# microsoft/XPretrain

Hardware: AMD Instinct MI355X
Metric: video-text pairs/sec (higher is better)
Workload: dtype bf16; 1 GPU; CLIP-ViP ViT-B/16 video-text contrastive train step (fwd+loss+bwd+grad-sync+clip+AdamW), 12 frames 224^2, 32 text tokens, local batch 8, BASELINE configs[1]; global_batch=8, parallelism=dp1, gemm_cu_budget=256, grad_wire=fp32, forced_one_rank_collectives=False, video_forward_chains=2, optimizer_overlaps_next_forward_from_layer=3, launch=eager

## Files before the change

include/xpretrain_hip.h:

```cpp
#ifndef XPRETRAIN_HIP_H
#define XPRETRAIN_HIP_H

#include <stddef.h>
#include <stdint.h>

#ifdef __cplusplus
extern "C" {
#endif

#define XP_ABI_VERSION 1

enum { XP_BF16 = 0, XP_F32 = 1 };
enum { XP_OK = 0, XP_ERR_ARG = -1, XP_ERR_LAUNCH = -2, XP_ERR_UNSUPPORTED = -3 };

int xp_abi_version(void);
const char* xp_last_error(void);

enum {
  XP_EPI_NONE = 0,
  XP_EPI_BIAS = 1,
  XP_EPI_BIAS_QSCALE = 2,
  XP_EPI_BIAS_GELU = 3,
  XP_EPI_BIAS_RESID = 4,
  XP_EPI_GELU_BWD = 5,
// ... 321 lines not shown
  const float* ln1_w; const float* ln1_b; const float* bqkv; const float* bo;
  const float* ln2_w; const float* ln2_b; const float* b1; const float* b2;
  void* h1; void* kv; float* mean1; float* rstd1;
  void* h1p; void* q; void* attn_o; void* x2; void* h2; void* pre; void* act; void* x3;
  float* mean1p; float* rstd1p; float* mean2; float* rstd2; float* stats;
  void* workspace; size_t workspace_bytes;
  const float* side_in; float* side_out; float* side_x2;
} XpLayerPooledFwd;
size_t xp_encoder_layer_pooled_fwd_workspace_bytes(const XpLayerDims* dims);
int xp_encoder_layer_pooled_fwd(const XpLayerPooledFwd* args, void* stream);

typedef struct XpLayerPooledBwd {
  XpLayerDims dims;
  const void* x; const void* h1; const void* kv; const void* h1p; const void* q; const void* attn_o; const void* x2;
  const void* h2; const void* pre; const void* act; const void* Wqkv; const void* Wo; const void* W1; const void* W2;
  const float* ln1_w; const float* ln2_w; const float* mean1; const float* rstd1; const float* mean1p; const float* rstd1p;
  const float* mean2; const float* rstd2; const float* stats;
  const void* dx3;
  void* dx;
  float* dln1_w; float* dln1_b; float* dwqkv; float* dbqkv; float* dwo; float* dbo;
  float* dln2_w; float* dln2_b; float* dw1; float* db1; float* dw2; float* db2;
  void* workspace; size_t workspace_bytes;
  const float* side_in; const float* side_x2;
} XpLayerPooledBwd;
size_t xp_encoder_layer_pooled_bwd_workspace_bytes(const XpLayerDims* dims);
int xp_encoder_layer_pooled_bwd(const XpLayerPooledBwd* args, void* stream);
void* xp_side_stream(void);

int xp_debug_set_gemm_trace(void* device_buffer);
int xp_debug_gemm_timer_arm(int64_t M, int64_t N, int64_t K, int32_t epilogue, int32_t a_kstrided, int32_t b_kstrided, int32_t split_k,
                            int32_t max_launches);
int32_t xp_debug_gemm_timer_read(float* ms, int32_t cap);
int xp_debug_set_attn_trace(void* device_buffer);
int xp_debug_gemm_occupancy(int lds_bytes);
enum { XP_GEMM_FAMILY_256 = 0,
       XP_GEMM_FAMILY_DIRECT = 1,
       XP_GEMM_FAMILY_STAGED = 2,
       XP_GEMM_FAMILY_FRAMES = 3 };
enum { XP_GEMM_EPI_FAST = 0,
       XP_GEMM_EPI_ROW8 = 1,
       XP_GEMM_EPI_ROW4 = 2 };
typedef struct XpGemmPlanInfo {
  int32_t family, tile_rows;
  int32_t split, flat_split;
  int64_t k_per_split;
  int32_t tiles_m, tiles_n, group_n;
  int32_t epi_impl;
  int32_t grid[3];
  int32_t reserved;
  int64_t colsum_rows;
} XpGemmPlanInfo;
int xp_debug_gemm_plan(const XpGemmDesc* desc, XpGemmPlanInfo* out);
enum { XP_ATTN_KERNEL_FWD = 0,
       XP_ATTN_KERNEL_FWD3 = 1,
       XP_ATTN_KERNEL_FWD4 = 2,
       XP_ATTN_KERNEL_BWD_PAIR = 3,
       XP_ATTN_KERNEL_BWD5 = 4,
       XP_ATTN_KERNEL_F32 = 5 };
enum { XP_ATTN_OPTIN_BWD6 = 6 };
typedef struct XpAttnPlanInfo {
  int32_t kernel;
  int32_t grid, lds_bytes;
  int32_t reduce_grid;
  int32_t uses_counter;
  int32_t reserved;
  int64_t part[2], delta[2], dq[2], dkv[2], counter[2];
// ... 43 lines not shown
```

xpretrain_amd/csrc/attention.hip:

```cpp
#include "common.h"
#include <math.h>
#include <stdlib.h>
#include <string.h>
#include <type_traits>

namespace {

constexpr int DH = 64;
constexpr float F32_MIN = -3.4028234663852886e38f;

struct AP {
  const bf16_t* qkv; int64_t ldqkv;
  bf16_t* out; const bf16_t* dout; int64_t ldo;
  bf16_t* dqkv;
  float* stats;
  const int64_t* pad;
  int mode, B, H, S, M, N, L, R;
  int nq, nprob;
  float q_scale;
  float* ws0; float* ws1; float* ws2;
  unsigned long long* tr;
  float* cs; int cs_main;
};

// ... 395 lines not shown
  }
}

template <int NTL>
__device__ __forceinline__ void fwd3_walk(FwdState (&st)[F3T], const AP& p, int frame, const char* gK, const char* gV,
                                          const bf16x8 (&qf)[F3T][2], int ng, int kb0, bool corner, int lane) {
  int t0 = 0;
  for (; t0 + 4 <= ng && kb0 + (t0 + 4) * 16 <= p.R; t0 += 4) fwd3_step<4, NTL, false>(st, p, frame, gK, gV, qf, t0, corner, lane, kb0);
  if (t0 < ng) {
    if (ng - t0 == 1) {
      if (kb0 + ng * 16 > p.R) fwd3_step<1, NTL, true>(st, p, frame, gK, gV, qf, t0, corner, lane, kb0);
      else                     fwd3_step<1, NTL, false>(st, p, frame, gK, gV, qf, t0, corner, lane, kb0);
    } else {
      fwd3_step<4, NTL, true>(st, p, frame, gK, gV, qf, t0, corner, lane, kb0);
    }
  }
}
__device__ __forceinline__ void fwd3_finish(const FwdState (&st)[F3T], const AP& p, const Prob& pr, int prob, int tile0, int nt,
                                            int wave, int lane) {
#pragma unroll
  for (int i = 0; i < F3T; ++i)
    if (i < nt) fwd_finish_row(st[i], p, pr, prob, (tile0 + wave + F3W * i) * 16 + (lane & 15), lane >> 4);
}
template <int NTL>
__device__ __forceinline__ void fwd3_problem(const AP& p, const Prob& pr, int prob, const char* gK, const char* gV,
                                             const bf16x8 (&qf)[F3T][2], int nsub, int wave, int lane) {
  FwdState st[F3T];
#pragma unroll
  for (int i = 0; i < F3T; ++i) fwd_init(st[i], M_INIT);
  fwd3_walk<NTL>(st, p, pr.n, gK, gV, qf, nsub, 0, wave == 0, lane);
  fwd3_finish(st, p, pr, prob, 0, NTL, wave, lane);
}

__global__ __launch_bounds__(F3THR, 2) void attn_fwd3_kernel(AP p) {
  extern __shared__ __attribute__((aligned(16))) char smem[];
  const int tid = threadIdx.x, lane = tid & 63;
  const int wave = __builtin_amdgcn_readfirstlane(tid >> 6);
  const int nsub = (p.R + 15) / 16;
  const int nt = (nsub - wave + F3W - 1) / F3W;
  int prob = blockIdx.x;
  if (prob >= p.nprob) return;
  int cur = 0;
  bf16x8 qf[F3T][2], qn[F3T][2];
  {
    const Prob pr(p, prob);
    fwd3_stage_kv(smem, smem + FG * 128, p, pr, lane, wave, 0);
    fwd3_load_q(qf, p, pr, wave, lane, 0);
  }
  unsigned long long* tr = (p.tr && (int)blockIdx.x == (int)gridDim.x / 2 && (wave == 0 || wave == 7) && lane == 0)
                               ? p.tr + (wave ? 64 : 0) : nullptr;
  int it = 0;
  for (;;) {
    if (tr && it < 8) tr[it * 4 + 0] = __builtin_amdgcn_s_memtime();
    __syncthreads();
    if (tr && it < 8) tr[it * 4 + 1] = __builtin_amdgcn_s_memtime();
    const Prob pr(p, prob);
    const int next = prob + (int)gridDim.x;
    char* gK = smem + cur * F3_BUF;
    if (next < p.nprob) {
      const Prob pn(p, next);
      char* nK = smem + (cur ^ 1) * F3_BUF;
      fwd3_stage_kv(nK, nK + FG * 128, p, pn, lane, wave, 0);
      fwd3_load_q(qn, p, pn, wave, lane, 0);
    }
    if (tr && it < 8) tr[it * 4 + 2] = __builtin_amdgcn_s_memtime();
    if (nt == 2)      fwd3_problem<2>(p, pr, prob, gK, gK + FG * 128, qf, nsub, wave, lane);
    else if (nt == 1) fwd3_problem<1>(p, pr, prob, gK, gK + FG * 128, qf, nsub, wave, lane);
    if (tr && it < 8) tr[it * 4 + 3] = __builtin_amdgcn_s_memtime();
    ++it;
    if (next >= p.nprob) break;
#pragma unroll
    for (int i = 0; i < F3T; ++i)
#pragma unroll
      for (int kk = 0; kk < 2; ++kk) qf[i][kk] = qn[i][kk];
    prob = next; cur ^= 1;
  }
}

struct F4Stage { int prob, qb, kg; bool valid; };
__device__ __forceinline__ F4Stage f4_stage(const AP& p, int s, int nqb, int ngrp) {
  F4Stage st;
  const int step = s / ngrp;
  st.kg = s - step * ngrp;
  const int xcd = blockIdx.x & 7, j = blockIdx.x >> 3;
  const int quads_per_xcd = ((int)gridDim.x >> 3) / nqb;
  const int quad = j / nqb, role = j - quad * nqb;
  st.qb = (role + step) % nqb;
  st.prob = (step * quads_per_xcd + quad) * 8 + xcd;
  st.valid = quad < quads_per_xcd && st.prob < p.nprob;
  return st;
}

__global__ __launch_bounds__(F3THR, 2) void attn_fwd4_kernel(AP p) {
  extern __shared__ __attribute__((aligned(16))) char smem[];
  const int tid = threadIdx.x, lane = tid & 63;
  const int wave = __builtin_amdgcn_readfirstlane(tid >> 6);
  const int ntiles = (p.R + 15) / 16;
  const int nqb = (ntiles + 2 * F3W - 1) / (2 * F3W);
  const int ngrp = (ntiles + FG / 16 - 1) / (FG / 16);
  int s = 0, cur = 0;
  F4Stage sg = f4_stage(p, 0, nqb, ngrp);
  if (!sg.valid) return;
  bf16x8 qf[F3T][2], qn[F3T][2];
  {
    const Prob pr(p, sg.prob);
    fwd3_stage_kv(smem, smem + FG * 128, p, pr, lane, wave, 0);
    fwd3_load_q(qf, p, pr, wave, lane, sg.qb * 2 * F3W);
  }
  FwdState st[F3T];
// ... 660 lines not shown
}
__device__ __forceinline__ void b5_colsum_finish_dq(const AP& p, const Prob& pr, const float* red, int tid) {
  if (!(p.cs && tid < DH)) return;
  float* row = cs_row(p, pr, 0);
  b5_colsum_finish(red, row, tid);
  for (int blk = 1; blk < p.nq; ++blk)
    for (int j = 0; j < 3; ++j) row[(int64_t)blk * 3 * p.H * DH + j * p.H * DH + tid] = 0.f;
}
__device__ __forceinline__ void b5_colsum_finish_dkv(const AP& p, int prev, const float* red, int tid) {
  if (!(p.cs && prev >= 0 && tid < 2 * DH)) return;
  const Prob pv(p, prev);
  float* row = cs_row(p, pv, 0);
  if (tid < DH) b5_colsum_finish(red + B5W * DH, row + p.H * DH, tid);
  else          b5_colsum_finish(red + 2 * B5W * DH, row + 2 * p.H * DH, tid - DH);
}

template <int CROWS>
__device__ __forceinline__ void b5_own_constants(float (&c)[2], float (&nd)[2], const B5Own& w, float* sC, int tile0, int wave, int lane) {
#pragma unroll
  for (int i = 0; i < 2; ++i) {
    float dl = 0.f;
#pragma unroll
    for (int kk = 0; kk < 2; ++kk)
#pragma unroll
      for (int e = 0; e < 8; ++e) dl += (float)w.d[i][kk][e] * (float)w.o[i][kk][e];
    dl += shfl_xor_lane(dl, 16, lane);
    dl += shfl_xor_lane(dl, 32, lane);
    c[i] = -(w.m[i] + w.lg[i]); nd[i] = -dl;
    const int rq = (tile0 + wave + B5W * i) * 16 + (lane & 15);
    if ((lane >> 4) == 0 && rq < CROWS) { sC[rq] = c[i]; sC[CROWS + rq] = nd[i]; }
  }
}

__global__ __launch_bounds__(B5THR, 2) void attn_bwd5_kernel(AP p, int* counter) {
  extern __shared__ __attribute__((aligned(16))) char smem[];
  char* X = smem; char* Y = smem + 2 * B5_IMG;
  float* sC = reinterpret_cast<float*>(smem + B5_OFF_STATS);
  float* red = reinterpret_cast<float*>(smem + B5_OFF_RED);
  int* sNext = reinterpret_cast<int*>(smem + B5_OFF_NEXT);
  char* stg = smem + B5_OFF_STG + (threadIdx.x >> 6) * B5_STG_WAVE;
  const int tid0 = threadIdx.x, lane0 = tid0 & 63;
  const int wave = __builtin_amdgcn_readfirstlane(tid0 >> 6);
  const int nt = (p.R + 15) / 16;
  const int nsteps = (nt + 1) / 2;
  const bool active = wave < nt;
  int prob = blockIdx.x, prev = -1;
  if (prob >= p.nprob) return;
  if (tid0 < 4 * 16 * 8) *reinterpret_cast<u32x4*>(smem + (tid0 >> 7) * B5_IMG + FG * 128 + (tid0 & 127) * 16) = u32x4{0, 0, 0, 0};
  B5Own w;
  {
    const Prob pr(p, prob);
    for (int j = 0; j < B5_PIECES; ++j) b5_stage_kv<FG, B5_IMG>(X, p, pr, 0, j, lane0, wave);
    b5_load_own(w, p, pr, wave, lane0, 0);
  }
  unsigned long long* tr = (p.tr && (int)blockIdx.x == (int)gridDim.x / 2 && (wave == 0 || wave == 7) && lane0 == 0)
                               ? p.tr + (wave ? 64 : 0) : nullptr;
  int it = 0;
#define B5_STAMP(k) do { if (tr && it < 8) tr[it * 8 + (k)] = __builtin_amdgcn_s_memtime(); } while (0)
  for (;;) {
    B5_STAMP(0);
    int lane = lane0;
    asm volatile("" : "+v"(lane));
    int tid = wave * 64 + lane, i16 = lane & 15, g = lane >> 4;
    if (tid == 0) *sNext = counter ? atomicAdd(counter, 1) + (int)gridDim.x : prob + (int)gridDim.x;
    __syncthreads();
    B5_STAMP(1);
    const Prob pr(p, prob);
    b5_colsum_finish_dkv(p, prev, red, tid);
    const bool corner = wave == 0 && pr.n != 0;
    bf16x8 kf[2][2], vf[2][2];
    {
      float c1[2], nd1[2];
      b5_own_constants<B5_ROWS>(c1, nd1, w, sC, 0, wave, lane);
      f32x4 c4[2], nd4[2];
#pragma unroll
      for (int i = 0; i < 2; ++i) { c4[i] = f32x4{c1[i], c1[i], c1[i], c1[i]}; nd4[i] = f32x4{nd1[i], nd1[i], nd1[i], nd1[i]}; }
      f32x4 dq[2][4];
#pragma unroll
      for (int i = 0; i < 2; ++i)
#pragma unroll
        for (int dt = 0; dt < 4; ++dt) dq[i][dt] = f32x4{0, 0, 0, 0};
      B5_STAMP(2);
      const int nfull = p.R / 32 < nsteps ? p.R / 32 : nsteps;
      int st = 0;
      for (; st < nfull; ++st) {
        if (st < B5_PIECES) b5_stage_qdo<FG, B5_IMG>(Y, p, pr, 0, st, lane, wave);
        if (active) b5_dq_step<false>(dq, p, X + st * (32 * 128), w, c4, nd4, 2 * st, corner, lane);
      }
      if (st < nsteps) {
        if (st < B5_PIECES) b5_stage_qdo<FG, B5_IMG>(Y, p, pr, 0, st, lane, wave);
        if (active) b5_dq_step<true>(dq, p, X + st * (32 * 128), w, c4, nd4, 2 * st, corner, lane);
        ++st;
      }
      for (; st < B5_PIECES; ++st) b5_stage_qdo<FG, B5_IMG>(Y, p, pr, 0, st, lane, wave);
      B5_STAMP(3);
      if (wave == 0 && i16 < p.M && i16 < p.R) store_dq_partial(p, prob, i16, g, dq[0]);
      float cs[8];
      b5_store_tiles(dq, p.q_scale, stg, p.dqkv + (int64_t)pr.b * p.S * p.ldqkv + pr.h * DH, p, pr.n, wave, lane, cs, 0);
      if (p.cs) b5_colsum_wave(cs, red + wave * DH, lane, true);
#pragma unroll
      for (int i = 0; i < 2; ++i)
#pragma unroll
        for (int kk = 0; kk < 2; ++kk) {
          const int t = wave + B5W * i < B5_ROWS / 16 ? wave + B5W * i : B5_ROWS / 16 - 1;
          kf[i][kk] = frag_rows(X, t, kk, lane);
          vf[i][kk] = frag_rows(X + B5_IMG, t, kk, lane);
        }
    }
    B5_STAMP(4);
    __syncthreads();
    B5_STAMP(5);
    lane = lane0;
    asm volatile("" : "+v"(lane));
    tid = wave * 64 + lane; i16 = lane & 15; g = lane >> 4;
    const int next = *sNext;
    b5_colsum_finish_dq(p, pr, red, tid);
    {
      f32x4 dk[2][4], dv[2][4];
#pragma unroll
      for (int i = 0; i < 2; ++i)
#pragma unroll
        for (int dt = 0; dt < 4; ++dt) { dk[i][dt] = f32x4{0, 0, 0, 0}; dv[i][dt] = f32x4{0, 0, 0, 0}; }
      for (int st = 0; st < nsteps || st < B5_PIECES; ++st) {
        if (st < B5_PIECES && next < p.nprob) { const Prob pn(p, next); b5_stage_kv<FG, B5_IMG>(X, p, pn, 0, st, lane, wave); }
        if (active && st < nsteps) {
          unsigned yo = 2u * B5_IMG + (unsigned)st * (32 * 128), co = (unsigned)B5_OFF_STATS + (unsigned)st * (32 * 4);
          asm volatile("" : "+s"(yo), "+s"(co));
          b5_dkv_step(dk, dv, p, smem + yo, reinterpret_cast<const float*>(smem + co), kf, vf, 2 * st, corner, lane);
        }
      }
      B5_STAMP(6);
      if (next < p.nprob) { const Prob pn(p, next); b5_load_own(w, p, pn, wave, lane, 0); }
      if (wave == 0 && i16 < p.M && i16 < p.R) store_dkv_partial(p, prob, i16, g, dk[0], dv[0]);
      bf16_t* colbase = p.dqkv + (int64_t)pr.b * p.S * p.ldqkv + pr.h * DH;
      float cs[8];
      b5_store_tiles(dk, 1.0f, stg, colbase + (int64_t)p.H * DH, p, pr.n, wave, lane, cs, 0);
      if (p.cs) b5_colsum_wave(cs, red + (B5W + wave) * DH, lane, true);
      b5_store_tiles(dv, 1.0f, stg, colbase + (int64_t)2 * p.H * DH, p, pr.n, wave, lane, cs, 0);
      if (p.cs) b5_colsum_wave(cs, red + (2 * B5W + wave) * DH, lane, true);
    }
    B5_STAMP(7);
    ++it;
    prev = prob;
    if (next >= p.nprob) break;
    prob = next;
  }
#undef B5_STAMP
  if (p.cs) {
    __syncthreads();
    b5_colsum_finish_dkv(p, prev, red, tid0);
  }
}

constexpr int B6_G = 192;
constexpr int B6_IMG = B6_G * 128;
constexpr int B6_BUF = 2 * B6_IMG;
constexpr int B6_RMAX = 6 * B6_G;
constexpr int B6_BLK = 2 * B5W;
constexpr int B6_PIECES = B6_G / 64;
constexpr int B6_OFF_STATS = 2 * B6_BUF;
constexpr int B6_OFF_RED = B6_OFF_STATS + 2 * B6_RMAX * 4;
constexpr int B6_OFF_NEXT = B6_OFF_RED + 3 * B5W * DH * 4;
constexpr int B6_OFF_STG = B6_OFF_NEXT + 16;
constexpr int B6_LDS = B6_OFF_STG + B5W * B5_STG_WAVE;
static_assert(B6_LDS <= 160 * 1024, "attn_bwd6_kernel: LDS budget");

__device__ __forceinline__ void b6_stage(char* buf, const AP& p, const Prob& pr, int kind, int grp, int lane, int wave, int j) {
  if (kind == 0) b5_stage_kv<B6_G, B6_IMG>(buf, p, pr, grp * B6_G, j, lane, wave);
  else           b5_stage_qdo<B6_G, B6_IMG>(buf, p, pr, grp * B6_G, j, lane, wave);
}
__device__ __forceinline__ void b6_load_own_kv(bf16x8 (&kf)[2][2], bf16x8 (&vf)[2][2], const AP& p, const Prob& pr, int wave, int lane,
                                               int tile0) {
  const int i16 = lane & 15, g = lane >> 4;
  const __amdgpu_buffer_rsrc_t rs = rsrc_kv(p, pr);
#pragma unroll
  for (int i = 0; i < 2; ++i) {
    const int rk = (tile0 + wave + B5W * i) * 16 + i16;
    const unsigned o = rk < p.R ? (unsigned)tok_of(p, pr.n, rk) * (unsigned)(p.ldqkv * 2) + g * 16 : OOB;
#pragma unroll
    for (int kk = 0; kk < 2; ++kk) {
      kf[i][kk] = __builtin_bit_cast(bf16x8, __builtin_amdgcn_raw_buffer_load_b128(rs, o + kk * 64, 0, 0));
      vf[i][kk] = __builtin_bit_cast(bf16x8, __builtin_amdgcn_raw_buffer_load_b128(rs, o + kk * 64, v_off(p), 0));
    }
  }
}

__global__ __launch_bounds__(B5THR, 2) void attn_bwd6_kernel(AP p, int* counter) {
  extern __shared__ __attribute__((aligned(16))) char smem[];
  float* sC = reinterpret_cast<float*>(smem + B6_OFF_STATS);
  float* red = reinterpret_cast<float*>(smem + B6_OFF_RED);
  int* sNext = reinterpret_cast<int*>(smem + B6_OFF_NEXT);
  char* stg = smem + B6_OFF_STG + (threadIdx.x >> 6) * B5_STG_WAVE;
#define B6_LANE0 ((int)__builtin_amdgcn_mbcnt_hi(~0u, __builtin_amdgcn_mbcnt_lo(~0u, 0u)))
  const int wave = __builtin_amdgcn_readfirstlane((int)threadIdx.x >> 6);
  const int nt = (p.R + 15) / 16;
  const int nblk = (nt + B6_BLK - 1) / B6_BLK;
  const int ngrp = (p.R + B6_G - 1) / B6_G;
  int prob = blockIdx.x, prev = -1;
  if (prob >= p.nprob) return;
  unsigned cur = 0;
  {
    const Prob pr(p, prob);
    for (int j = 0; j < B6_PIECES; ++j) b6_stage(smem, p, pr, 0, 0, B6_LANE0, wave, j);
  }
  for (;;) {
    const Prob pr(p, prob);
    if (wave == 0 && B6_LANE0 == 0) *sNext = counter ? atomicAdd(counter, 1) + (int)gridDim.x : prob + (int)gridDim.x;
    bf16_t* colbase = p.dqkv + (int64_t)pr.b * p.S * p.ldqkv + pr.h * DH;
    for (int qb = 0; qb < nblk; ++qb) {
      const bool active = qb * B6_BLK + wave < nt;
      const bool corner = wave == 0 && pr.n != 0 && qb == 0;
      B5Own w;
      float c1[2], nd1[2];
      f32x4 dq[2][4];
      for (int kg = 0; kg < ngrp; ++kg) {
        int lane = B6_LANE0;
        asm volatile("" : "+v"(lane));
        const int tid = wave * 64 + lane;
        __syncthreads();
        if (qb == 0 && kg == 0) b5_colsum_finish_dkv(p, prev, red, tid);
        if (kg == 0) {
          b5_load_own(w, p, pr, wave, lane, qb * B6_BLK);
          b5_own_constants<B6_RMAX>(c1, nd1, w, sC, qb * B6_BLK, wave, lane);
#pragma unroll
          for (int i = 0; i < 2; ++i)
#pragma unroll
            for (int dt = 0; dt < 4; ++dt) dq[i][dt] = f32x4{0, 0, 0, 0};
        }
        const int nkind = kg + 1 < ngrp || qb + 1 < nblk ? 0 : 1, ngr = kg + 1 < ngrp ? kg + 1 : 0;
        char* nbuf = smem + (cur ^ (unsigned)B6_BUF);
        const int left = p.R - kg * B6_G;
        const int nsteps = left >= B6_G ? B6_G / 32 : (left + 31) / 32, nfull = left >= B6_G ? B6_G / 32 : left / 32;
#define B6_SPLAT_CONSTANTS                                                                                       \
  f32x4 c4[2], nd4[2];                                                                                           \
  _Pragma("unroll") for (int i = 0; i < 2; ++i) {                                                                \
    float c = c1[i], n = nd1[i];                                                                                 \
    asm volatile("" : "+v"(c), "+v"(n));                                                                         \
    c4[i] = f32x4{c, c, c, c}; nd4[i] = f32x4{n, n, n, n};                                                       \
  }
        int st = 0;
        for (; st < nfull; ++st) {
          if (st < B6_PIECES) b6_stage(nbuf, p, pr, nkind, ngr, lane, wave, st);
          if (active) {
            unsigned xo = cur + (unsigned)st * (32 * 128);
            asm volatile("" : "+s"(xo));
            B6_SPLAT_CONSTANTS;
            b5_dq_step<false, B6_IMG>(dq, p, smem + xo, w, c4, nd4, kg * (B6_G / 16) + 2 * st, corner, lane);
          }
        }
        if (st < nsteps) {
          if (st < B6_PIECES) b6_stage(nbuf, p, pr, nkind, ngr, lane, wave, st);
          if (active) {
            unsigned xo = cur + (unsigned)st * (32 * 128);
            asm volatile("" : "+s"(xo));
            B6_SPLAT_CONSTANTS;
            b5_dq_step<true, B6_IMG>(dq, p, smem + xo, w, c4, nd4, kg * (B6_G / 16) + 2 * st, corner, lane);
          }
          ++st;
        }
#undef B6_SPLAT_CONSTANTS
        for (; st < B6_PIECES; ++st) b6_stage(nbuf, p, pr, nkind, ngr, lane, wave, st);
        cur ^= (unsigned)B6_BUF;
      }
      int lane = B6_LANE0;
      asm volatile("" : "+v"(lane));
      const int i16 = lane & 15, g = lane >> 4;
      if (qb == 0 && wave == 0 && i16 < p.M) store_dq_partial(p, prob, i16, g, dq[0]);
      float cs[8];
      b5_store_tiles(dq, p.q_scale, stg, colbase, p, pr.n, wave, lane, cs, qb * B6_BLK);
      if (p.cs) b5_colsum_wave(cs, red + wave * DH, lane, qb == 0);
    }
    int next = p.nprob;
    for (int kb = 0; kb < nblk; ++kb) {
      const bool active = kb * B6_BLK + wave < nt;
      const bool corner = wave == 0 && pr.n != 0 && kb == 0;
      bf16x8 kf[2][2], vf[2][2];
      f32x4 dk[2][4], dv[2][4];
      for (int qg = 0; qg < ngrp; ++qg) {
        int lane = B6_LANE0;
        asm volatile("" : "+v"(lane));
        const int tid = wave * 64 + lane;
        __syncthreads();
        if (kb == 0 && qg == 0) {
          next = __builtin_amdgcn_readfirstlane(*sNext);
          b5_colsum_finish_dq(p, pr, red, tid);
        }
        if (qg == 0) {
          b6_load_own_kv(kf, vf, p, pr, wave, lane, kb * B6_BLK);
#pragma unroll
          for (int i = 0; i < 2; ++i)
#pragma unroll
            for (int dt = 0; dt < 4; ++dt) { dk[i][dt] = f32x4{0, 0, 0, 0}; dv[i][dt] = f32x4{0, 0, 0, 0}; }
        }
        const bool last = qg + 1 == ngrp && kb + 1 == nblk;
        const bool more = !last || next < p.nprob;
        const Prob pn(p, last && more ? next : prob);
        const int nkind = last ? 0 : 1, ngr = qg + 1 < ngrp ? qg + 1 : 0;
        char* nbuf = smem + (cur ^ (unsigned)B6_BUF);
        const int left = p.R - qg * B6_G;
        const int nsteps = left >= B6_G ? B6_G / 32 : (left + 31) / 32;
        for (int st = 0; st < nsteps || st < B6_PIECES; ++st) {
          if (st < B6_PIECES && more) b6_stage(nbuf, p, pn, nkind, ngr, lane, wave, st);
          if (active && st < nsteps) {
            unsigned yo = cur + (unsigned)st * (32 * 128), co = (unsigned)B6_OFF_STATS + (unsigned)(qg * B6_G + st * 32) * 4;
            asm volatile("" : "+s"(yo), "+s"(co));
            b5_dkv_step<B6_IMG, B6_RMAX>(dk, dv, p, smem + yo, reinterpret_cast<const float*>(smem + co), kf, vf,
                                         qg * (B6_G / 16) + 2 * st, corner, lane);
          }
        }
        cur ^= (unsigned)B6_BUF;
      }
      int lane = B6_LANE0;
      asm volatile("" : "+v"(lane));
      const int i16 = lane & 15, g = lane >> 4;
      if (kb == 0 && wave == 0 && i16 < p.M) store_dkv_partial(p, prob, i16, g, dk[0], dv[0]);
      float cs[8];
      b5_store_tiles(dk, 1.0f, stg, colbase + (int64_t)p.H * DH, p, pr.n, wave, lane, cs, kb * B6_BLK);
// ... 67 lines not shown
  const unsigned per_cu = (unsigned)(P < cus ? P : cus);
  if (!c.bwd && persistent && R <= FG) {
    p.kernel = XP_ATTN_KERNEL_FWD3; p.grid = per_cu; p.lds = F3_LDS; p.lds_kernel = reinterpret_cast<const void*>(attn_fwd3_kernel);
  } else if (!c.bwd && persistent && cus % 8 == 0 && cus / 8 >= cdiv(cdiv(R, 16), 2 * F3W)) {
    p.kernel = XP_ATTN_KERNEL_FWD4; p.grid = (unsigned)cus; p.lds = F3_LDS; p.lds_kernel = reinterpret_cast<const void*>(attn_fwd4_kernel);
  } else if (c.bwd && persistent && R <= FG && !xp_debug_flag("attn_bwd_split")) {
    p.kernel = XP_ATTN_KERNEL_BWD5; p.grid = per_cu; p.lds = B5_LDS; p.lds_kernel = reinterpret_cast<const void*>(attn_bwd5_kernel);
    p.uses_counter = true;
  } else if (c.bwd && persistent && R > FG && R <= B6_RMAX && g_attn_bwd_wide && !xp_debug_flag("attn_bwd_split")) {
    p.kernel = XP_ATTN_OPTIN_BWD6; p.grid = per_cu; p.lds = B6_LDS; p.lds_kernel = reinterpret_cast<const void*>(attn_bwd6_kernel);
    p.uses_counter = true;
  } else {
    p.kernel = c.bwd ? XP_ATTN_KERNEL_BWD_PAIR : XP_ATTN_KERNEL_FWD; p.grid = (unsigned)(cdiv(P, 8) * 8 * nq);
  }
  p.reduce_grid = proxy ? (unsigned)(c.B * c.H * c.M) : 0;
  return p;
}

int plan_attn_for(const AttnCall& c, int cus, AttnPlan& p) {
  const bool device = cus <= 0;
  if (device && !(cus = xp_device_cus())) return XP_ERR_LAUNCH;
  p = plan_attn(c, cus);
  return device && p.lds && !xp_device_cus(p.lds_kernel, p.lds) ? XP_ERR_LAUNCH : XP_OK;
}

}

int xp_attn_f32_fwd(const void* qkv, int64_t ldqkv, void* out, int64_t ldo, float* stats, const int64_t* pad, int32_t mode,
                    int64_t B, int64_t H, int64_t S, int64_t M, int64_t N, int64_t L, hipStream_t st);
int xp_attn_f32_bwd(const void* qkv, int64_t ldqkv, const void* out, const void* dout, int64_t ldo, const float* stats,
                    const int64_t* pad, void* dqkv, float q_scale, int32_t mode, int64_t B, int64_t H, int64_t S,
                    int64_t M, int64_t N, int64_t L, float* delta_ws, hipStream_t st);

static void* g_attn_trace = nullptr;
extern "C" int xp_debug_set_attn_trace(void* device_buffer) { g_attn_trace = device_buffer; return XP_OK; }

extern "C" int xp_set_attn_bwd_wide(int32_t on) { g_attn_bwd_wide = on != 0; return XP_OK; }
extern "C" int32_t xp_get_attn_bwd_wide(void) { return g_attn_bwd_wide; }

extern "C" size_t xp_attn_workspace_bytes(int32_t mode, int64_t B, int64_t H, int64_t M, int64_t N, int64_t L) {
  const int64_t fwd = plan_attn(AttnCall{mode, B, H, M + N * L, M, N, L, XP_BF16, false, false}, 0).ws_bytes;
  const int64_t bwd = plan_attn(AttnCall{mode, B, H, M + N * L, M, N, L, XP_BF16, false, true}, 0).ws_bytes;
  return (size_t)(fwd > bwd ? fwd : bwd);
}

extern "C" int xp_attn_fwd(const void* qkv, int64_t ldqkv, void* out, int64_t ldo, float* stats,
                           const int64_t* pad_mask, int32_t mode, int64_t B, int64_t H, int64_t S,
                           int64_t M, int64_t N, int64_t L, int32_t dtype,
                           void* workspace, size_t workspace_bytes, void* stream) {
  XP_REQUIRE(qkv && out && stats, "xp_attn_fwd: null pointer");
  if (mode == XP_ATTN_CAUSAL) { M = 0; N = 1; L = S; }
  int rc = check_common("xp_attn_fwd", mode, B, H, S, M, N, L, ldqkv, ldo, dtype);
  if (rc) return rc;
  if (dtype == XP_F32) return xp_attn_f32_fwd(qkv, ldqkv, out, ldo, stats, pad_mask, mode, B, H, S, M, N, L, (hipStream_t)stream);
  XP_REQUIRE(mode == XP_ATTN_CAUSAL || (workspace && workspace_bytes >= xp_attn_workspace_bytes(mode, B, H, M, N, L)),
             "xp_attn_fwd: workspace too small");
  AttnPlan pl;
  if ((rc = plan_attn_for(AttnCall{mode, B, H, S, M, N, L, dtype, pad_mask != nullptr, false}, 0, pl))) return rc;
  AP p = pl.geo;
  p.qkv = (const bf16_t*)qkv; p.ldqkv = ldqkv; p.out = (bf16_t*)out; p.ldo = ldo; p.stats = stats; p.pad = pad_mask;
  p.ws0 = pl.part.in(workspace); p.tr = reinterpret_cast<unsigned long long*>(g_attn_trace);
  hipStream_t st = (hipStream_t)stream;
  if (pl.kernel == XP_ATTN_KERNEL_FWD3)      attn_fwd3_kernel<<<pl.grid, F3THR, pl.lds, st>>>(p);
  else if (pl.kernel == XP_ATTN_KERNEL_FWD4) attn_fwd4_kernel<<<pl.grid, F3THR, pl.lds, st>>>(p);
  else                                       attn_fwd_kernel<<<pl.grid, FTHR, 0, st>>>(p);
  XP_CHECK_LAUNCH("xp_attn_fwd");
  if (pl.reduce_grid) {
    attn_fwd_merge_kernel<<<pl.reduce_grid, 256, 0, st>>>(p);
    XP_CHECK_LAUNCH("xp_attn_fwd(merge)");
  }
  return XP_OK;
}

extern "C" int64_t xp_attn_bwd_colsum_rows(int32_t mode, int64_t B, int64_t H, int64_t S, int64_t M, int64_t N, int64_t L, int32_t dtype) {
  return plan_attn(AttnCall{mode, B, H, S, M, N, L, dtype, false, true}, 0).colsum_rows;
}

extern "C" int xp_attn_bwd(const void* qkv, int64_t ldqkv, const void* out, const void* dout, int64_t ldo,
                           const float* stats, const int64_t* pad_mask, void* dqkv, float q_scale,
                           int32_t mode, int64_t B, int64_t H, int64_t S, int64_t M, int64_t N, int64_t L, int32_t dtype,
                           void* workspace, size_t workspace_bytes, void* stream) {
  return xp_attn_bwd2(qkv, ldqkv, out, dout, ldo, stats, pad_mask, dqkv, q_scale, mode, B, H, S, M, N, L, dtype, workspace,
                      workspace_bytes, nullptr, stream);
}

extern "C" int xp_attn_bwd2(const void* qkv, int64_t ldqkv, const void* out, const void* dout, int64_t ldo,
                            const float* stats, const int64_t* pad_mask, void* dqkv, float q_scale,
                            int32_t mode, int64_t B, int64_t H, int64_t S, int64_t M, int64_t N, int64_t L, int32_t dtype,
                            void* workspace, size_t workspace_bytes, float* dqkv_colsum_partials, void* stream) {
  XP_REQUIRE(qkv && out && dout && stats && dqkv, "xp_attn_bwd: null pointer");
  XP_REQUIRE(!dqkv_colsum_partials || xp_attn_bwd_colsum_rows(mode, B, H, S, M, N, L, dtype) > 0,
             "xp_attn_bwd2: fused column sums are not available for this problem (xp_attn_bwd_colsum_rows() == 0)");
  if (mode == XP_ATTN_CAUSAL) { M = 0; N = 1; L = S; }
  int rc = check_common("xp_attn_bwd", mode, B, H, S, M, N, L, ldqkv, ldo, dtype);
  if (rc) return rc;
  XP_REQUIRE(workspace && workspace_bytes >= xp_attn_workspace_bytes(mode, B, H, M, N, L), "xp_attn_bwd: workspace too small");
  if (dtype == XP_F32)
    return xp_attn_f32_bwd(qkv, ldqkv, out, dout, ldo, stats, pad_mask, dqkv, q_scale, mode, B, H, S, M, N, L, (float*)workspace,
                           (hipStream_t)stream);
  AttnPlan pl;
  if ((rc = plan_attn_for(AttnCall{mode, B, H, S, M, N, L, dtype, pad_mask != nullptr, true}, 0, pl))) return rc;
  AP p = pl.geo;
  p.qkv = (const bf16_t*)qkv; p.ldqkv = ldqkv; p.out = (bf16_t*)out; p.dout = (const bf16_t*)dout; p.ldo = ldo;
  p.dqkv = (bf16_t*)dqkv; p.stats = const_cast<float*>(stats); p.pad = pad_mask; p.q_scale = q_scale;
  p.ws0 = pl.delta.in(workspace); p.ws1 = pl.dq.in(workspace); p.ws2 = pl.dkv.in(workspace);
  p.cs = dqkv_colsum_partials; p.tr = reinterpret_cast<unsigned long long*>(g_attn_trace);
  hipStream_t st = (hipStream_t)stream;
  int* counter = reinterpret_cast<int*>(pl.counter.in(workspace));
  if (pl.uses_counter && hipMemsetAsync(counter, 0, sizeof(int), st) != hipSuccess) { xp_set_error("xp_attn_bwd: counter reset failed"); return XP_ERR_LAUNCH; }
  if (pl.kernel == XP_ATTN_KERNEL_BWD5) {
    attn_bwd5_kernel<<<pl.grid, B5THR, pl.lds, st>>>(p, counter);
    XP_CHECK_LAUNCH("xp_attn_bwd(fused)");
  } else if (pl.kernel == XP_ATTN_OPTIN_BWD6) {
    attn_bwd6_kernel<<<pl.grid, B5THR, pl.lds, st>>>(p, counter);
    XP_CHECK_LAUNCH("xp_attn_bwd(fused, wide)");
  } else {
    attn_bwd_dq_kernel<<<pl.grid, FTHR, 0, st>>>(p);
    XP_CHECK_LAUNCH("xp_attn_bwd(dq)");
    attn_bwd_dkv_kernel<<<pl.grid, FTHR, 0, st>>>(p);
    XP_CHECK_LAUNCH("xp_attn_bwd(dkv)");
  }
  if (pl.reduce_grid) {
    attn_bwd_proxy_reduce_kernel<<<pl.reduce_grid, 256, 0, st>>>(p);
    XP_CHECK_LAUNCH("xp_attn_bwd(proxy reduce)");
  }
  return XP_OK;
}

extern "C" int xp_debug_attn_plan(int32_t mode, int64_t B, int64_t H, int64_t S, int64_t M, int64_t N, int64_t L, int32_t dtype,
                                  int32_t has_pad_mask, int32_t backward, int32_t cus, XpAttnPlanInfo* out) {
  XP_REQUIRE(out, "xp_debug_attn_plan: null argument");
  AttnPlan p;
  const int rc = plan_attn_for(AttnCall{mode, B, H, S, M, N, L, dtype, has_pad_mask != 0, backward != 0}, cus, p);
  if (rc) return rc;
  *out = XpAttnPlanInfo{p.kernel, (int32_t)p.grid, p.lds, (int32_t)p.reduce_grid, p.uses_counter, 0, {p.part.off, p.part.bytes},
                        {p.delta.off, p.delta.bytes}, {p.dq.off, p.dq.bytes}, {p.dkv.off, p.dkv.bytes},
                        {p.counter.off, p.counter.bytes}, p.ws_bytes, p.colsum_rows};
  return XP_OK;
}
```

xpretrain_amd/csrc/common.cpp:

```cpp
#include "common.h"
#include <string.h>
#include <map>
#include <mutex>

static thread_local char g_err[512] = "";

void xp_set_error(const char* fmt, ...) {
  va_list ap;
  va_start(ap, fmt);
  vsnprintf(g_err, sizeof(g_err), fmt, ap);
  va_end(ap);
}

extern "C" const char* xp_last_error(void) { return g_err; }

bool xp_debug_flag(const char* name) {
  const char* env = getenv("XPRETRAIN_DEBUG");
  if (!env || !*env) return false;
  const size_t n = strlen(name);
  for (const char* p = env; (p = strstr(p, name)) != nullptr; p += n) {
    const bool left = p == env || p[-1] == ',', right = p[n] == '\0' || p[n] == ',';
    if (left && right) return true;
  }
  return false;
}
extern "C" int xp_abi_version(void) { return XP_ABI_VERSION; }

int xp_device_cus(const void* kernel, int lds_bytes) {
  static std::mutex mu;
  static std::map<std::pair<const void*, int>, int> known;
  int dev = -1, n = 0;
  if (hipGetDevice(&dev) != hipSuccess || dev < 0) { xp_set_error("no current HIP device"); return 0; }
  std::lock_guard<std::mutex> lock(mu);
  int& cus = known[{kernel, dev}];
  if (!cus && kernel && hipFuncSetAttribute(kernel, hipFuncAttributeMaxDynamicSharedMemorySize, lds_bytes) != hipSuccess) cus = -1;
  if (!cus) cus = hipDeviceGetAttribute(&n, hipDeviceAttributeMultiprocessorCount, dev) == hipSuccess && n > 0 ? n : 256;
  if (cus < 0) xp_set_error("device %d refused a kernel's dynamic-LDS opt-in of %d bytes", dev, lds_bytes);
  return cus > 0 ? cus : 0;
}
```

xpretrain_amd/csrc/common.h:

```cpp
#pragma once
#include <hip/hip_runtime.h>
#include <stdint.h>
#include <stdio.h>
#include <stdarg.h>
#include "../../include/xpretrain_hip.h"

typedef __bf16 bf16_t;
typedef __attribute__((ext_vector_type(8))) __bf16 bf16x8;
typedef __attribute__((ext_vector_type(4))) __bf16 bf16x4;
typedef __attribute__((ext_vector_type(2))) __bf16 bf16x2;
typedef __attribute__((ext_vector_type(4))) float f32x4;
typedef __attribute__((ext_vector_type(2))) float f32x2;
typedef __attribute__((ext_vector_type(4))) short i16x4;
typedef __attribute__((ext_vector_type(4))) unsigned int u32x4;
typedef __attribute__((ext_vector_type(2))) unsigned int u32x2;

void xp_set_error(const char* fmt, ...);
bool xp_debug_flag(const char* name);
int xp_device_cus(const void* kernel = nullptr, int lds_bytes = 0);

#define XP_REQUIRE(cond, ...)                                  \
  do {                                                         \
    if (!(cond)) { xp_set_error(__VA_ARGS__); return XP_ERR_ARG; } \
  } while (0)

#define XP_CHECK_LAUNCH(name)                                                   \
  do {                                                                          \
    hipError_t e__ = hipGetLastError();                                         \
    if (e__ != hipSuccess) {                                                    \
      xp_set_error("%s: launch failed: %s", name, hipGetErrorString(e__));      \
      return XP_ERR_LAUNCH;                                                     \
    }                                                                           \
  } while (0)

static inline int64_t cdiv(int64_t a, int64_t b) { return (a + b - 1) / b; }

void xp_launch_rows_reduce(const float* in, float* out, int nrows, int nsum, int width, int accumulate, hipStream_t st);

void xp_launch_small_gemm(const float* X, int64_t sxi, int64_t sxk, const float* Y, int64_t syk, int64_t syj, float* C, int64_t ldc,
                          int I, int J, int K, const float* log_scale, int accumulate, hipStream_t st);
void xp_launch_logits(const float* vis, const float* txt, float* A, int64_t n, int64_t d, const float* log_scale, hipStream_t st);

template <typename T> struct DT;
template <> struct DT<bf16_t> { static constexpr int id = XP_BF16; };
template <> struct DT<float>  { static constexpr int id = XP_F32; };

__device__ __forceinline__ float to_f(float x) { return x; }
__device__ __forceinline__ float to_f(bf16_t x) { return (float)x; }
template <typename T> __device__ __forceinline__ T from_f(float x);
template <> __device__ __forceinline__ float from_f<float>(float x) { return x; }
template <> __device__ __forceinline__ bf16_t from_f<bf16_t>(float x) { return (bf16_t)x; }

__device__ __forceinline__ f32x4 load4(const float* p) { return *reinterpret_cast<const f32x4*>(p); }
__device__ __forceinline__ f32x4 load4(const bf16_t* p) {
  bf16x4 v = *reinterpret_cast<const bf16x4*>(p);
  return f32x4{(float)v[0], (float)v[1], (float)v[2], (float)v[3]};
}
__device__ __forceinline__ void store4(float* p, f32x4 v) { *reinterpret_cast<f32x4*>(p) = v; }
__device__ __forceinline__ void store4(bf16_t* p, f32x4 v) {
  bf16x4 o = {(bf16_t)v[0], (bf16_t)v[1], (bf16_t)v[2], (bf16_t)v[3]};
  *reinterpret_cast<bf16x4*>(p) = o;
}

struct f32x8 { f32x4 lo, hi; };
__device__ __forceinline__ f32x8 load8(const float* p) { return f32x8{load4(p), load4(p + 4)}; }
__device__ __forceinline__ f32x8 load8(const bf16_t* p) {
  const bf16x8 v = *reinterpret_cast<const bf16x8*>(p);
  return f32x8{f32x4{(float)v[0], (float)v[1], (float)v[2], (float)v[3]}, f32x4{(float)v[4], (float)v[5], (float)v[6], (float)v[7]}};
// ... 81 lines not shown
```

xpretrain_amd/hip_ops.py:

```python
from __future__ import annotations

import ctypes as C
import functools
import math
from typing import NamedTuple, Optional

import torch

from . import _lib as L

_DT = {torch.bfloat16: L.XP_BF16, torch.float32: L.XP_F32}


def _stream():
    return C.c_void_p(torch.cuda.current_stream().cuda_stream)


def _p(t: Optional[torch.Tensor]):
    return C.c_void_p(0 if t is None else t.data_ptr())


def _dt(t: torch.Tensor) -> int:
    try:
        return _DT[t.dtype]
# ... 690 lines not shown
    return out, stats


def attn_probs(qkv: torch.Tensor, stats: torch.Tensor, B: int, S: int, H: int, *, size=None, pad_mask=None, out=None):
    _chk(qkv, "qkv"); _chk(stats, "stats", torch.float32)
    mode = L.ATTN_PROXY if size is not None else L.ATTN_CAUSAL
    M, N, Lp = size if size is not None else (0, 1, S)
    if stats.numel() != B * H * S * 2 or not stats.is_contiguous() or not qkv.is_contiguous() or qkv.numel() != B * S * 3 * H * 64:
        raise ValueError("attn_probs: qkv must be a contiguous [B*S, 3*H*64] matrix and stats attn_fwd's contiguous [B,H,S,2]")
    if pad_mask is not None:
        _chk(pad_mask, "pad_mask", torch.int64)
    shapes = ((B, H, M, S), (B, H, N, Lp, M + Lp)) if size is not None else ((B, H, S, S),)
    outs = (out,) if isinstance(out, torch.Tensor) else tuple(out) if out is not None else (None,) * len(shapes)
    if len(outs) != len(shapes):
        raise ValueError(f"attn_probs: out must be {'the (proxy, frame) pair' if size is not None else 'one tensor'}")
    bufs = [_dest("attn_probs", t, nm, torch.float32, shp, qkv.device) for t, shp, nm in zip(outs, shapes, ("out[0]", "out[1]"))]
    frame, proxy = (bufs[1], bufs[0]) if size is not None else (bufs[0], None)
    L.check(L.lib().xp_attn_probs(_p(qkv), 3 * H * 64, _p(stats), _p(pad_mask), _p(frame), _p(proxy), mode, B, H, S, M, N, Lp,
                                  _dt(qkv), _stream()), "xp_attn_probs")
    return (proxy, frame) if size is not None else frame


def attn_plan(B: int, S: int, H: int, *, size=None, pad_mask=None, dtype=torch.bfloat16, backward=False, cus=0) -> dict:
    mode = L.ATTN_PROXY if size is not None else L.ATTN_CAUSAL
    M, N, Lp = size if size is not None else (0, 1, S)
    info = L.XpAttnPlanInfo()
    L.check(L.lib().xp_debug_attn_plan(mode, B, H, S, M, N, Lp, _DT[dtype], int(pad_mask is not None), int(backward), cus,
                                       C.byref(info)), "xp_debug_attn_plan")
    plan = {f: getattr(info, f) for f, _ in info._fields_ if f != "reserved"}
    plan.update({f: tuple(plan[f]) for f in ("part", "delta", "dq", "dkv", "counter")}, kernel=L.ATTN_OPTIN_KERNELS.get(info.kernel) or L.ATTN_KERNELS[info.kernel])
    return plan


def set_attn_bwd_wide(on: bool) -> None:
    L.check(L.lib().xp_set_attn_bwd_wide(int(bool(on))), "xp_set_attn_bwd_wide")


def get_attn_bwd_wide() -> bool:
    return bool(L.lib().xp_get_attn_bwd_wide())


def attn_bwd(qkv, out, dout, stats, B, S, H, *, size=None, pad_mask=None, q_scale=1.0, colsum_defer=None,
             colsum_name="dbqkv", colsum_out=None):
    mode = L.ATTN_PROXY if size is not None else L.ATTN_CAUSAL
    M, N, Lp = size if size is not None else (0, 1, S)
    dqkv = torch.empty_like(qkv)
    ws = _attn_ws(mode, B, H, M, N, Lp, qkv.device)
    nrows = int(L.lib().xp_attn_bwd_colsum_rows(mode, B, H, S, M, N, Lp, _dt(qkv))) if colsum_defer is not None else 0
    part = colsum_defer.slot(nrows * 3 * H * 64 * 4, colsum_name) if nrows else None
    L.check(L.lib().xp_attn_bwd2(_p(qkv), 3 * H * 64, _p(out), _p(dout), H * 64, _p(stats), _p(pad_mask), _p(dqkv),
                                 float(q_scale), mode, B, H, S, M, N, Lp, _dt(qkv), _p(ws), ws.numel(), _p(part), _stream()),
            "xp_attn_bwd")
    if colsum_defer is None:
        return dqkv
    if not nrows:
        return dqkv, colsum_deferred(dqkv, B * S, 3 * H * 64, colsum_defer, name=colsum_name, out=colsum_out)
    cs = torch.empty(3 * H * 64, dtype=torch.float32, device=qkv.device) if colsum_out is None else colsum_out
    colsum_defer.add(part, 0, cs, nrows, 3 * H * 64, 3 * H * 64)
    return dqkv, cs


def _rows_ld(t: torch.Tensor, name: str, width: int) -> int:
    _chk(t, name)
    if t.dim() != 2 or t.stride(1) != 1 or t.shape[1] < width:
        raise TypeError(f"{name}: expected a [rows, >= {width}] matrix with contiguous rows, got {tuple(t.shape)} strides {t.stride()}")
    return t.stride(0)
# ... 165 lines not shown
```

Before: 566.8 pairs/s.

## Use self-resetting per-stream atomic work slots for attention fwd and bwd scheduling

```diff
diff --git a/include/xpretrain_hip.h b/include/xpretrain_hip.h
--- a/include/xpretrain_hip.h
+++ b/include/xpretrain_hip.h
@@ -377,6 +377,7 @@
                             int32_t max_launches);
 int32_t xp_debug_gemm_timer_read(float* ms, int32_t cap);
 int xp_debug_set_attn_trace(void* device_buffer);
+int xp_debug_attn_slot(void* stream, int32_t* host_out);
 int xp_debug_gemm_occupancy(int lds_bytes);
 enum { XP_GEMM_FAMILY_256 = 0,
        XP_GEMM_FAMILY_DIRECT = 1,
diff --git a/xpretrain_amd/csrc/attention.hip b/xpretrain_amd/csrc/attention.hip
--- a/xpretrain_amd/csrc/attention.hip
+++ b/xpretrain_amd/csrc/attention.hip
@@ -451,20 +451,41 @@
   fwd3_finish(st, p, pr, prob, 0, NTL, wave, lane);
 }
 
-__global__ __launch_bounds__(F3THR, 2) void attn_fwd3_kernel(AP p) {
+__device__ __forceinline__ int slot_fetch(int* slot) { return atomicAdd(slot, 1) + (int)gridDim.x; }
+__device__ __forceinline__ int slot_release_begin(int* slot) {
+  __builtin_amdgcn_fence(__ATOMIC_RELEASE, "workgroup");
+  return atomicAdd(slot + 1, 1);
+}
+__device__ __forceinline__ void slot_release_end(int* slot, int released_before) {
+  if (released_before == (int)gridDim.x - 1) {
+    __hip_atomic_store(slot, 0, __ATOMIC_RELAXED, __HIP_MEMORY_SCOPE_AGENT);
+    __hip_atomic_store(slot + 1, 0, __ATOMIC_RELAXED, __HIP_MEMORY_SCOPE_AGENT);
+  }
+}
+__device__ __forceinline__ void slot_release(int* slot) { slot_release_end(slot, slot_release_begin(slot)); }
+
+__global__ __launch_bounds__(F3THR, 2) void attn_fwd3_kernel(AP p, int* slot) {
   extern __shared__ __attribute__((aligned(16))) char smem[];
+  __shared__ int sNext[2];
   const int tid = threadIdx.x, lane = tid & 63;
   const int wave = __builtin_amdgcn_readfirstlane(tid >> 6);
+#define lane0 (wave == 0 && __builtin_amdgcn_mbcnt_hi(~0u, __builtin_amdgcn_mbcnt_lo(~0u, 0u)) == 0)
   const int nsub = (p.R + 15) / 16;
   const int nt = (nsub - wave + F3W - 1) / F3W;
   int prob = blockIdx.x;
-  if (prob >= p.nprob) return;
+  if (prob >= p.nprob) {
+    if (slot && lane0) slot_release(slot);
+    return;
+  }
   int cur = 0;
+  int fetched = 0;
+  if (slot && lane0) fetched = slot_fetch(slot);
   bf16x8 qf[F3T][2], qn[F3T][2];
   {
     const Prob pr(p, prob);
     fwd3_stage_kv(smem, smem + FG * 128, p, pr, lane, wave, 0);
     fwd3_load_q(qf, p, pr, wave, lane, 0);
+    if (slot && lane0) sNext[0] = fetched;
   }
   unsigned long long* tr = (p.tr && (int)blockIdx.x == (int)gridDim.x / 2 && (wave == 0 || wave == 7) && lane == 0)
                                ? p.tr + (wave ? 64 : 0) : nullptr;
@@ -474,13 +495,16 @@
     __syncthreads();
     if (tr && it < 8) tr[it * 4 + 1] = __builtin_amdgcn_s_memtime();
     const Prob pr(p, prob);
-    const int next = prob + (int)gridDim.x;
+    const int next = __builtin_amdgcn_readfirstlane(slot ? sNext[cur] : prob + (int)gridDim.x);
     char* gK = smem + cur * F3_BUF;
     if (next < p.nprob) {
       const Prob pn(p, next);
       char* nK = smem + (cur ^ 1) * F3_BUF;
       fwd3_stage_kv(nK, nK + FG * 128, p, pn, lane, wave, 0);
       fwd3_load_q(qn, p, pn, wave, lane, 0);
+      if (slot && lane0) fetched = slot_fetch(slot);
+    } else if (slot && lane0) {
+      fetched = slot_release_begin(slot);
     }
     if (tr && it < 8) tr[it * 4 + 2] = __builtin_amdgcn_s_memtime();
     if (nt == 2)      fwd3_problem<2>(p, pr, prob, gK, gK + FG * 128, qf, nsub, wave, lane);
@@ -488,12 +512,15 @@
     if (tr && it < 8) tr[it * 4 + 3] = __builtin_amdgcn_s_memtime();
     ++it;
     if (next >= p.nprob) break;
+    if (slot && lane0) sNext[cur ^ 1] = fetched;
 #pragma unroll
     for (int i = 0; i < F3T; ++i)
 #pragma unroll
       for (int kk = 0; kk < 2; ++kk) qf[i][kk] = qn[i][kk];
     prob = next; cur ^= 1;
   }
+  if (slot && lane0) slot_release_end(slot, fetched);
+#undef lane0
 }
 
 struct F4Stage { int prob, qb, kg; bool valid; };
@@ -1220,7 +1247,7 @@
   }
 }
 
-__global__ __launch_bounds__(B5THR, 2) void attn_bwd5_kernel(AP p, int* counter) {
+__global__ __launch_bounds__(B5THR, 2) void attn_bwd5_kernel(AP p, int* counter, int slot) {
   extern __shared__ __attribute__((aligned(16))) char smem[];
   char* X = smem; char* Y = smem + 2 * B5_IMG;
   float* sC = reinterpret_cast<float*>(smem + B5_OFF_STATS);
@@ -1233,7 +1260,10 @@
   const int nsteps = (nt + 1) / 2;
   const bool active = wave < nt;
   int prob = blockIdx.x, prev = -1;
-  if (prob >= p.nprob) return;
+  if (prob >= p.nprob) {
+    if (slot && tid0 == 0) slot_release(counter);
+    return;
+  }
   if (tid0 < 4 * 16 * 8) *reinterpret_cast<u32x4*>(smem + (tid0 >> 7) * B5_IMG + FG * 128 + (tid0 & 127) * 16) = u32x4{0, 0, 0, 0};
   B5Own w;
   {
@@ -1243,16 +1273,17 @@
   }
   unsigned long long* tr = (p.tr && (int)blockIdx.x == (int)gridDim.x / 2 && (wave == 0 || wave == 7) && lane0 == 0)
                                ? p.tr + (wave ? 64 : 0) : nullptr;
-  int it = 0;
+  int it = 0, released = 0;
 #define B5_STAMP(k) do { if (tr && it < 8) tr[it * 8 + (k)] = __builtin_amdgcn_s_memtime(); } while (0)
   for (;;) {
     B5_STAMP(0);
     int lane = lane0;
     asm volatile("" : "+v"(lane));
     int tid = wave * 64 + lane, i16 = lane & 15, g = lane >> 4;
-    if (tid == 0) *sNext = counter ? atomicAdd(counter, 1) + (int)gridDim.x : prob + (int)gridDim.x;
     __syncthreads();
     B5_STAMP(1);
+    int fetched = prob + (int)gridDim.x;
+    if (tid == 0 && counter) fetched = slot_fetch(counter);
     const Prob pr(p, prob);
     b5_colsum_finish_dkv(p, prev, red, tid);
     const bool corner = wave == 0 && pr.n != 0;
@@ -1296,12 +1327,14 @@
         }
     }
     B5_STAMP(4);
+    if (tid == 0) *sNext = fetched;
     __syncthreads();
     B5_STAMP(5);
     lane = lane0;
     asm volatile("" : "+v"(lane));
     tid = wave * 64 + lane; i16 = lane & 15; g = lane >> 4;
     const int next = *sNext;
+    if (slot && next >= p.nprob && tid == 0) released = slot_release_begin(counter);
     b5_colsum_finish_dq(p, pr, red, tid);
     {
       f32x4 dk[2][4], dv[2][4];
@@ -1338,6 +1371,7 @@
     __syncthreads();
     b5_colsum_finish_dkv(p, prev, red, tid0);
   }
+  if (slot && tid0 == 0) slot_release_end(counter, released);
 }
 
 constexpr int B6_G = 192;
@@ -1373,7 +1407,7 @@
   }
 }
 
-__global__ __launch_bounds__(B5THR, 2) void attn_bwd6_kernel(AP p, int* counter) {
+__global__ __launch_bounds__(B5THR, 2) void attn_bwd6_kernel(AP p, int* counter, int slot) {
   extern __shared__ __attribute__((aligned(16))) char smem[];
   float* sC = reinterpret_cast<float*>(smem + B6_OFF_STATS);
   float* red = reinterpret_cast<float*>(smem + B6_OFF_RED);
@@ -1385,7 +1419,10 @@
   const int nblk = (nt + B6_BLK - 1) / B6_BLK;
   const int ngrp = (p.R + B6_G - 1) / B6_G;
   int prob = blockIdx.x, prev = -1;
-  if (prob >= p.nprob) return;
+  if (prob >= p.nprob) {
+    if (slot && threadIdx.x == 0) slot_release(counter);
+    return;
+  }
   unsigned cur = 0;
   {
     const Prob pr(p, prob);
@@ -1393,7 +1430,7 @@
   }
   for (;;) {
     const Prob pr(p, prob);
-    if (wave == 0 && B6_LANE0 == 0) *sNext = counter ? atomicAdd(counter, 1) + (int)gridDim.x : prob + (int)gridDim.x;
+    int fetched = prob + (int)gridDim.x;
     bf16_t* colbase = p.dqkv + (int64_t)pr.b * p.S * p.ldqkv + pr.h * DH;
     for (int qb = 0; qb < nblk; ++qb) {
       const bool active = qb * B6_BLK + wave < nt;
@@ -1407,6 +1444,7 @@
         const int tid = wave * 64 + lane;
         __syncthreads();
         if (qb == 0 && kg == 0) b5_colsum_finish_dkv(p, prev, red, tid);
+        if (qb + 1 == nblk && kg + 1 == ngrp && tid == 0 && counter) fetched = slot_fetch(counter);
         if (kg == 0) {
           b5_load_own(w, p, pr, wave, lane, qb * B6_BLK);
           b5_own_constants<B6_RMAX>(c1, nd1, w, sC, qb * B6_BLK, wave, lane);
@@ -1458,6 +1496,7 @@
       b5_store_tiles(dq, p.q_scale, stg, colbase, p, pr.n, wave, lane, cs, qb * B6_BLK);
       if (p.cs) b5_colsum_wave(cs, red + wave * DH, lane, qb == 0);
     }
+    if (wave == 0 && B6_LANE0 == 0) *sNext = fetched;
     int next = p.nprob;
     for (int kb = 0; kb < nblk; ++kb) {
       const bool active = kb * B6_BLK + wave < nt;
@@ -1471,6 +1510,7 @@
         __syncthreads();
         if (kb == 0 && qg == 0) {
           next = __builtin_amdgcn_readfirstlane(*sNext);
+          if (slot && next >= p.nprob && tid == 0) slot_release(counter);
           b5_colsum_finish_dq(p, pr, red, tid);
         }
         if (qg == 0) {
@@ -1604,6 +1644,20 @@
                     const int64_t* pad, void* dqkv, float q_scale, int32_t mode, int64_t B, int64_t H, int64_t S,
                     int64_t M, int64_t N, int64_t L, float* delta_ws, hipStream_t st);
 
+static bool attn_static(bool bwd) { return xp_debug_flag("attn_static") || xp_debug_flag(bwd ? "attn_static=bwd" : "attn_static=fwd"); }
+
+extern "C" int xp_debug_attn_slot(void* stream, int32_t* out) {
+  XP_REQUIRE(out, "xp_debug_attn_slot: null argument");
+  int index = -1, v[XP_SLOT_INTS] = {0, 0};
+  const int* slot = xp_attn_slot((hipStream_t)stream, &index);
+  if (slot && (hipStreamSynchronize((hipStream_t)stream) != hipSuccess || hipMemcpy(v, slot, sizeof v, hipMemcpyDeviceToHost) != hipSuccess)) {
+    xp_set_error("xp_debug_attn_slot: reading the slot failed: %s", hipGetErrorString(hipGetLastError()));
+    return XP_ERR_LAUNCH;
+  }
+  out[0] = index; out[1] = v[0]; out[2] = v[1];
+  return XP_OK;
+}
+
 static void* g_attn_trace = nullptr;
 extern "C" int xp_debug_set_attn_trace(void* device_buffer) { g_attn_trace = device_buffer; return XP_OK; }
 
@@ -1633,7 +1687,7 @@
   p.qkv = (const bf16_t*)qkv; p.ldqkv = ldqkv; p.out = (bf16_t*)out; p.ldo = ldo; p.stats = stats; p.pad = pad_mask;
   p.ws0 = pl.part.in(workspace); p.tr = reinterpret_cast<unsigned long long*>(g_attn_trace);
   hipStream_t st = (hipStream_t)stream;
-  if (pl.kernel == XP_ATTN_KERNEL_FWD3)      attn_fwd3_kernel<<<pl.grid, F3THR, pl.lds, st>>>(p);
+  if (pl.kernel == XP_ATTN_KERNEL_FWD3)      attn_fwd3_kernel<<<pl.grid, F3THR, pl.lds, st>>>(p, attn_static(false) ? nullptr : xp_attn_slot(st));
   else if (pl.kernel == XP_ATTN_KERNEL_FWD4) attn_fwd4_kernel<<<pl.grid, F3THR, pl.lds, st>>>(p);
   else                                       attn_fwd_kernel<<<pl.grid, FTHR, 0, st>>>(p);
   XP_CHECK_LAUNCH("xp_attn_fwd");
@@ -1678,13 +1732,14 @@
   p.ws0 = pl.delta.in(workspace); p.ws1 = pl.dq.in(workspace); p.ws2 = pl.dkv.in(workspace);
   p.cs = dqkv_colsum_partials; p.tr = reinterpret_cast<unsigned long long*>(g_attn_trace);
   hipStream_t st = (hipStream_t)stream;
-  int* counter = reinterpret_cast<int*>(pl.counter.in(workspace));
-  if (pl.uses_counter && hipMemsetAsync(counter, 0, sizeof(int), st) != hipSuccess) { xp_set_error("xp_attn_bwd: counter reset failed"); return XP_ERR_LAUNCH; }
+  int* slot = pl.uses_counter && !attn_static(true) ? xp_attn_slot(st) : nullptr;
+  int* counter = slot ? slot : reinterpret_cast<int*>(pl.counter.in(workspace));
+  if (pl.uses_counter && !slot && hipMemsetAsync(counter, 0, sizeof(int), st) != hipSuccess) { xp_set_error("xp_attn_bwd: counter reset failed"); return XP_ERR_LAUNCH; }
   if (pl.kernel == XP_ATTN_KERNEL_BWD5) {
-    attn_bwd5_kernel<<<pl.grid, B5THR, pl.lds, st>>>(p, counter);
+    attn_bwd5_kernel<<<pl.grid, B5THR, pl.lds, st>>>(p, counter, slot != nullptr);
     XP_CHECK_LAUNCH("xp_attn_bwd(fused)");
   } else if (pl.kernel == XP_ATTN_OPTIN_BWD6) {
-    attn_bwd6_kernel<<<pl.grid, B5THR, pl.lds, st>>>(p, counter);
+    attn_bwd6_kernel<<<pl.grid, B5THR, pl.lds, st>>>(p, counter, slot != nullptr);
     XP_CHECK_LAUNCH("xp_attn_bwd(fused, wide)");
   } else {
     attn_bwd_dq_kernel<<<pl.grid, FTHR, 0, st>>>(p);
diff --git a/xpretrain_amd/csrc/common.cpp b/xpretrain_amd/csrc/common.cpp
--- a/xpretrain_amd/csrc/common.cpp
+++ b/xpretrain_amd/csrc/common.cpp
@@ -26,6 +26,29 @@
 }
 extern "C" int xp_abi_version(void) { return XP_ABI_VERSION; }
 
+int* xp_attn_slot(hipStream_t st, int* index) {
+  static std::mutex mu;
+  static XpSlotTable table;
+  static int* page[XP_SLOT_DEVICES];
+  if (index) *index = -1;
+  int dev = -1;
+  if (hipGetDevice(&dev) != hipSuccess || dev < 0 || dev >= XP_SLOT_DEVICES) { (void)hipGetLastError(); return nullptr; }
+  std::lock_guard<std::mutex> lock(mu);
+  if (!page[dev]) {
+    static const int zeros[XP_SLOTS * XP_SLOT_INTS] = {};
+    hipStreamCaptureStatus cap = hipStreamCaptureStatusNone;
+    int* p = nullptr;
+    bool good = hipStreamIsCapturing(st, &cap) == hipSuccess && cap == hipStreamCaptureStatusNone;
+    good = good && hipMalloc(reinterpret_cast<void**>(&p), sizeof zeros) == hipSuccess;
+    if (good && hipMemcpy(p, zeros, sizeof zeros, hipMemcpyHostToDevice) != hipSuccess) { (void)hipFree(p); good = false; }
+    if (!good) { (void)hipGetLastError(); return nullptr; }
+    page[dev] = p;
+  }
+  const int i = table.take(dev, st);
+  if (index) *index = i;
+  return i < 0 ? nullptr : page[dev] + i * XP_SLOT_INTS;
+}
+
 int xp_device_cus(const void* kernel, int lds_bytes) {
   static std::mutex mu;
   static std::map<std::pair<const void*, int>, int> known;
diff --git a/xpretrain_amd/csrc/common.h b/xpretrain_amd/csrc/common.h
--- a/xpretrain_amd/csrc/common.h
+++ b/xpretrain_amd/csrc/common.h
@@ -34,6 +34,29 @@
   } while (0)
 
 static inline int64_t cdiv(int64_t a, int64_t b) { return (a + b - 1) / b; }
+
+constexpr int XP_SLOT_DEVICES = 16, XP_SLOTS = 16, XP_SLOT_INTS = 2;
+struct XpSlotKeys {
+  const void* key[XP_SLOTS];
+  int n;
+  int find(const void* stream) const {
+    for (int i = 0; i < n; ++i)
+      if (key[i] == stream) return i;
+    return -1;
+  }
+  int take(const void* stream) {
+    const int i = find(stream);
+    if (i >= 0 || n == XP_SLOTS) return i;
+    key[n] = stream;
+    return n++;
+  }
+};
+struct XpSlotTable {
+  XpSlotKeys dev[XP_SLOT_DEVICES];
+  int take(int device, const void* stream) { return device < 0 || device >= XP_SLOT_DEVICES ? -1 : dev[device].take(stream); }
+  int find(int device, const void* stream) const { return device < 0 || device >= XP_SLOT_DEVICES ? -1 : dev[device].find(stream); }
+};
+int* xp_attn_slot(hipStream_t st, int* index = nullptr);
 
 void xp_launch_rows_reduce(const float* in, float* out, int nrows, int nsum, int width, int accumulate, hipStream_t st);
 
diff --git a/xpretrain_amd/hip_ops.py b/xpretrain_amd/hip_ops.py
--- a/xpretrain_amd/hip_ops.py
+++ b/xpretrain_amd/hip_ops.py
@@ -746,6 +746,13 @@
     return plan
 
 
+def attn_slot(stream=None):
+    out = (C.c_int32 * 3)()
+    st = _stream() if stream is None else C.c_void_p(stream.cuda_stream)
+    L.check(L.lib().xp_debug_attn_slot(st, out), "xp_debug_attn_slot")
+    return tuple(out)
+
+
 def set_attn_bwd_wide(on: bool) -> None:
     L.check(L.lib().xp_set_attn_bwd_wide(int(bool(on))), "xp_set_attn_bwd_wide")
 
```

Result: no change. 565.3 pairs/s (-0.3%).
